# jimonld2000/AudioDenoiser

Hardware: AMD Instinct MI355X
Metric: spectrogram frames/sec (forward), 513x256 fp32 (higher is better)
Workload: dtype f32; 1 GPU; BASELINE configs[1]: batch=64 synthetic 513x256 fp32 spectrograms on one MI355X, full U-Net forward + per-clip perceptual loss; batch_per_gpu=64, global_batch=64, freq_bins=513, frames=256, parallelism=clips sharded over 1 rank(s), weights replicated, no data-path collective, lib_digest=ac1cc53c7748

## Files before the change

audiodenoiser_amd/csrc/adn_internal.h:

```cpp
#pragma once
#include <hip/hip_runtime.h>
#include <atomic>
#include <cstddef>
#include <cstdint>
#include <type_traits>

namespace adn {

template <typename T> constexpr int ACT_BLOCK = 32 / (int)sizeof(T);
template <typename T>
__host__ __device__ __forceinline__ long act_off(int C, long HW, long pix, int c)
{
    constexpr int B = ACT_BLOCK<T>;
    (void)C;
    return ((long)(c / B) * HW + pix) * B + (c % B);
}

#ifdef __HIPCC__
typedef float f32x2 __attribute__((ext_vector_type(2)));
typedef float f32x4 __attribute__((ext_vector_type(4)));
typedef float f32x16 __attribute__((ext_vector_type(16)));
typedef _Float16 f16x2 __attribute__((ext_vector_type(2)));
typedef _Float16 f16x4 __attribute__((ext_vector_type(4)));
typedef _Float16 f16x8 __attribute__((ext_vector_type(8)));
// ... 158 lines not shown
{
    const double out_mb = (double)out_floats * 4.0 * 1e-6;
    int best = 1;
    double tbest = 0.0;
    for (int ks = 1; ks <= ADN_MAX_KSPLIT; ks *= 2) {
        if (nchunk % ks || (ks > 1 && nchunk / ks < 8)) break;
        const double t = 8.0 + 1.28 * (nchunk / ks) * (double)((nwg * ks + 767) / 768) + (ks > 1 ? 4.0 + (ks + 1) * out_mb / 8.0 : 0.0);
        if (ks == 1 || t < tbest - 0.5) {
            best = ks;
            tbest = t;
        }
    }
    return best;
}

inline int conv16_ksplit(long nwg, int nchunk, size_t out_floats)
{
    if (nwg > 64) return 1;
    int ks = 1;
    while (ks < 8 && nwg * ks * 2 <= 256 && nchunk % (ks * 2) == 0 && nchunk / (ks * 2) >= 4 &&
           (size_t)(ks * 2) * out_floats * 4 <= ((size_t)32 << 20))
        ks *= 2;
    return ks;
}

enum ConvKind { CONV3X3_RELU = 0, CONV3X3_RELU_POOL = 1, CONVT2X2 = 2, CONV3X3_RELU_DOT = 3, WINO_GEMM = 4 };

struct ConvGeom {
    int TH;
    int BN;
    int KC;
};
ConvGeom conv_geom(ConvKind kind, int Cout, bool f16);
long conv_mfma_tiles(ConvKind kind, bool f16, ConvArgs &a);

template <auto... KERNELS>
hipError_t lds_opt_in(size_t bytes)
{
    static std::atomic<unsigned long long> done{0};
    int dev = 0;
    if (hipGetDevice(&dev) != hipSuccess) return hipErrorInvalidDevice;
    const unsigned long long bit = 1ull << (dev & 63);
    if (done.load(std::memory_order_acquire) & bit) return hipSuccess;
    for (const void *k : {reinterpret_cast<const void *>(KERNELS)...}) {
        const hipError_t e = hipFuncSetAttribute(k, hipFuncAttributeMaxDynamicSharedMemorySize, (int)bytes);
        if (e != hipSuccess) return e;
    }
    done.fetch_or(bit, std::memory_order_release);
    return hipSuccess;
}
inline int device_cus()
{
    static std::atomic<int> cus{0};
    int c = cus.load(std::memory_order_relaxed);
    if (c == 0) {
        int dev = 0;
        if (hipGetDevice(&dev) != hipSuccess || hipDeviceGetAttribute(&c, hipDeviceAttributeMultiprocessorCount, dev) != hipSuccess || c < 8)
            return 0;
        c &= ~7;
        cus.store(c, std::memory_order_relaxed);
    }
    return c;
}

hipError_t launch_conv_mfma(ConvKind kind, const ConvArgs &a, bool f16, hipStream_t st);
hipError_t launch_conv_reduce(ConvKind kind, const ConvArgs &a, bool f16, hipStream_t st);
hipError_t launch_convt_reduce(const float *partial, const float *bias, float *out, int ksplit, int N, int Ho, int Wo, int Cout,
                               hipStream_t st);
constexpr int WINO_BN = 32;
hipError_t launch_wino_conv(ConvKind kind, const ConvArgs &a, hipStream_t st);
long wino_tiles(ConvArgs &a);
bool wino4_applicable(ConvKind kind, const ConvArgs &a, bool force);
long wino4_workgroups(const ConvArgs &a);
hipError_t launch_wino4_conv(ConvKind kind, const ConvArgs &a, hipStream_t st);

struct Wino3sGeom {
    int tilesY, tilesX;
    long rows;
    size_t v_bytes, m_bytes;
    long gemm_grid;
};
bool wino3s_applicable(ConvKind kind, const ConvArgs &a);
Wino3sGeom wino3s_geom(const ConvArgs &a);
hipError_t launch_wino3s_conv(ConvKind kind, const ConvArgs &a, float *V, float *M, hipStream_t st);
hipError_t launch_wino_gemm(const float *V, const void *U, float *M, long rows, int Cin, int Cout, hipStream_t st);

bool conv16_applicable(ConvKind kind, const ConvArgs &a);
hipError_t launch_conv16(ConvKind kind, const ConvArgs &a, bool resident, hipStream_t st);

bool convt16_applicable(const ConvArgs &a);
hipError_t launch_convt16(const ConvArgs &a, hipStream_t st);

hipError_t launch_conv_first(const float *x, const float *w9x64, const float *bias, void *out, bool f16,
                             int N, int H, int W, int Cin, hipStream_t st);
hipError_t launch_dot_finish(const float *planes, int nplanes, float bias, float *y, long npix, hipStream_t st);
hipError_t launch_conv_out(const void *in, bool f16, const float *w64, float bias, float *out, long npix, long HW,
                           long out_stride, hipStream_t st);
hipError_t launch_nhwc_to_nchw(const void *in, bool f16, float *out, int N, int H, int W, int C, hipStream_t st);

hipError_t launch_stft_mag(const float *audio, int n_clips, long L, int n_fft, int hop, int center, long n_frames,
                           float *out, int rows, long row_stride, long clip_stride, int quantize, hipStream_t st);
constexpr hipError_t ADN_COLD_IN_CAPTURE = hipErrorStreamCaptureUnsupported;
bool stream_is_capturing(hipStream_t st);
hipError_t stft_tables(int n_fft, const float **out, hipStream_t st);
hipError_t loss_tables(hipStream_t st);
hipError_t launch_gl_polar(const float *mag, const float *rnd, int n_clips, int F, int T, void *spec, hipStream_t st);
hipError_t launch_istft_frames(const void *spec, int n_clips, int T, int n_fft, float *buf, hipStream_t st);
hipError_t launch_istft_ola(const float *buf, int n_clips, int T, int n_fft, int hop, float *audio, hipStream_t st);
hipError_t launch_stft_complex(const float *audio, int n_clips, long L, int n_fft, int hop, int T, void *spec,
                               hipStream_t st);
struct DenoiseGeom {
    int T, K, Wd, S, V;
};
bool denoise_geom(int n_frames, int window, int overlap, DenoiseGeom *g);
hipError_t launch_denoise_windows(const void *spec, int n_clips, int F, const DenoiseGeom &g, float *out, hipStream_t st);
hipError_t launch_denoise_stitch(const float *y, int n_clips, int F, const DenoiseGeom &g, int clamp, float *out,
                                 hipStream_t st);
hipError_t launch_denoise_resynth(const float *y, const void *spec, int n_clips, long L, int n_fft, int hop,
                                  const DenoiseGeom &g, float *audio, hipStream_t st);
struct SpectralConsts {
    float smooth, one_minus_smooth, beta, gamma, growth, alpha, one_minus_alpha, gain_floor, bias;
};
hipError_t launch_spectral_gain(const void *spec, int n_clips, int T, int F, const SpectralConsts &k, const float *state_in,
                                float *state_out, float *out, int width, int col0, hipStream_t st);
constexpr int SPECTRAL_MAX_ROWS = 256;
struct SpectralRow {
    int slot, fresh;
};
struct SpectralRows {
    int n;
    SpectralRow row[SPECTRAL_MAX_ROWS];
};
hipError_t launch_spectral_gain_windows(const float *windows, float *y, int n_rows, int n_steps, int F, int W, int col0, int n_cols,
                                        const SpectralConsts &k, float *state, const SpectralRows &rows, hipStream_t st);
struct WpeConsts {
    int K, D, I;
    float loading, rho;
};
long wpe_grid(int n_clips, int F, int K);
hipError_t launch_wpe(const void *spec, int n_clips, int T, int F, const WpeConsts &k, void *spec_out, float *mag_out, int width,
                      hipStream_t st);
struct StreamGeom {
    int n_fft, hop, W, B, A;
    int S, RX, RM;
    long x_off, mag_off, hist_off, tail_off, total;
};
struct StreamCall {
    int first, n_steps, T, L;
    int base, end, f_new0, f_new1;
    int slot_in, slot_out;
    int f_first, f_last, p_begin, p_first, p_out, p_tail, p_end;
};
__host__ __device__ inline StreamCall stream_call_of(const StreamGeom &g, long first, int n_steps, long final_length)
{
    StreamCall c;
    const long B = g.B, D = g.B + g.A, hop = g.hop, M = g.n_fft / 2, keep = g.n_fft - g.hop;
    const long last = first + n_steps - 1;
    c.first = (int)first;
    c.n_steps = n_steps;
    c.T = -1;
    c.L = -1;
    bool closes = false;
    if (final_length > 0) {
        const long T = 1 + final_length / hop, K = (T + B - 1) / B;
        c.T = (int)T;
        c.L = (int)final_length;
        closes = last == K - 1;
    }
// ... 117 lines not shown
```

audiodenoiser_amd/csrc/conv_kernels.hip:

```cpp
#include "adn_internal.h"

#include <cstdlib>

namespace adn {

namespace {

constexpr int TW = 16;
constexpr int CONVT_KG = 2, CONVT_WPE = 4;

template <typename T> struct Elem;
template <> struct Elem<float> { static constexpr int EPV = 4; };
template <> struct Elem<_Float16> { static constexpr int EPV = 8; };

template <int TH, int BN, int WM, int WN>
__device__ __forceinline__ void conv_epilogue_raw(const ConvArgs &p, f32x16 (&acc)[TH * TW / 32 / WM][BN / 32 / WN], int lane, int wave,
                                                  int ct, int n, int ty, int tx)
{
    constexpr int MB = TH * TW / 32 / WM, NB = BN / 32 / WN;
    const int wm = wave / WN, wn = wave % WN;
    const int hh = lane >> 5, l31 = lane & 31;
    float *ob = static_cast<float *>(p.out) + (size_t)n * p.H * p.W * p.Cout;
#pragma unroll
    for (int j = 0; j < NB; ++j) {
// ... 804 lines not shown
        for (int s = 1; s < ADN_MAX_KSPLIT; ++s)
            if (s < ksplit) v += t[s];
        v += bv;
        v.x = relu_nan(v.x); v.y = relu_nan(v.y); v.z = relu_nan(v.z); v.w = relu_nan(v.w);
        *reinterpret_cast<Tx4 *>(out + (size_t)n * img + act_off<T>(Cout, (long)H * W, (long)gy * W + gx, c4)) = as_t(v);
        return v;
    };
    if constexpr (!POOL) {
        finish(by, bx);
    } else {
        f32x4 mx = {0.f, 0.f, 0.f, 0.f};
#pragma unroll
        for (int a = 0; a < 2; ++a)
#pragma unroll
            for (int b = 0; b < 2; ++b) {
                const int gy = 2 * by + a, gx = 2 * bx + b;
                if (gy >= H || gx >= W) continue;
                const f32x4 v = finish(gy, gx);
                mx.x = max_nan(mx.x, v.x); mx.y = max_nan(mx.y, v.y); mx.z = max_nan(mx.z, v.z); mx.w = max_nan(mx.w, v.w);
            }
        if (by < H / 2 && bx < W / 2)
            *reinterpret_cast<Tx4 *>(pool + (size_t)n * (H / 2) * (W / 2) * Cout +
                                     act_off<T>(Cout, (long)(H / 2) * (W / 2), (long)by * (W / 2) + bx, c4)) = as_t(mx);
    }
}

template <typename T>
hipError_t launch_conv_mfma_t(ConvKind kind, const ConvArgs &a, hipStream_t st)
{
    if constexpr (sizeof(T) == 2) {
        if (a.ksplit > 1) {
            if (kind != CONV3X3_RELU) return hipErrorInvalidValue;
            return launch_dma_cfg<T, 32, 64, 8, 1, 9, 1, CONV3X3_RELU, 4, 0, 1>(a, st);
        }
        if (kind == CONVT2X2) return launch_dma_cfg<T, 8, 128, 2, 2, 1, CONVT_KG, CONVT2X2, CONVT_WPE>(a, st);
        if (kind == CONV3X3_RELU_DOT) {
            if (a.nct != 1 || !a.dotw || !a.dot_out) return hipErrorInvalidValue;
            return launch_dma_cfg<T, 32, 64, 8, 1, 9, 1, CONV3X3_RELU_DOT, 4>(a, st);
        }
        if (kind == CONV3X3_RELU_POOL) return launch_dma_cfg<T, 32, 64, 8, 1, 9, 1, CONV3X3_RELU_POOL, 4>(a, st);
        return launch_dma_cfg<T, 32, 64, 8, 1, 9, 1, CONV3X3_RELU, 4>(a, st);
    } else {
        if (kind == CONV3X3_RELU_DOT) return hipErrorInvalidValue;
        if (kind == CONVT2X2) {
            if (a.split && a.ksplit > 1) return launch_dma_cfg<T, 8, 128, 2, 2, 1, CONVT_KG, CONVT2X2, 3, 1, 1>(a, st);
            if (a.ksplit > 1) return hipErrorInvalidValue;
            if (a.split) return launch_dma_cfg<T, 8, 128, 2, 2, 1, CONVT_KG, CONVT2X2, 3, 1>(a, st);
            return launch_dma_cfg<T, 8, 128, 2, 2, 1, CONVT_KG, CONVT2X2, CONVT_WPE>(a, st);
        }
        if (a.Cout == 64) {
            if (kind == CONV3X3_RELU_POOL) return launch_cfg<T, 16, 64, 4, 1, 9, 1, CONV3X3_RELU_POOL>(a, st);
            return launch_cfg<T, 16, 64, 4, 1, 9, 1, CONV3X3_RELU>(a, st);
        }
        if (kind == CONV3X3_RELU_POOL) return launch_cfg<T, 8, 128, 2, 2, 9, 1, CONV3X3_RELU_POOL>(a, st);
        return launch_cfg<T, 8, 128, 2, 2, 9, 1, CONV3X3_RELU>(a, st);
    }
}

}

ConvGeom conv_geom(ConvKind kind, int Cout, bool f16)
{
    const int cpg = f16 ? 16 : 8;
    if (kind == CONVT2X2) return ConvGeom{8, 128, CONVT_KG * cpg};
    if (f16) return ConvGeom{32, 64, cpg};
    if (Cout == 64) return ConvGeom{16, 64, cpg};
    return ConvGeom{8, 128, cpg};
}

long conv_mfma_tiles(ConvKind kind, bool f16, ConvArgs &a)
{
    const ConvGeom g = conv_geom(kind, a.Cout, f16);
    a.tilesY = (a.H + g.TH - 1) / g.TH;
    a.tilesX = (a.W + TW - 1) / TW;
    a.nct = (kind == CONVT2X2 ? 4 * a.Cout : a.Cout) / g.BN;
    return conv_workgroups(a);
}

hipError_t launch_conv_mfma(ConvKind kind, const ConvArgs &a, bool f16, hipStream_t st)
{
    return f16 ? launch_conv_mfma_t<_Float16>(kind, a, st) : launch_conv_mfma_t<float>(kind, a, st);
}

hipError_t launch_wino_gemm(const float *V, const void *U, float *M, long rows, int Cin, int Cout, hipStream_t st)
{
    if (!V || !U || !M || rows < 1 || rows >= (1L << 25) || Cin < 16 || (Cin & 15) || Cout < 128 || (Cout & 127)) return hipErrorInvalidValue;
    ConvArgs a{};
    a.N = 36;
    a.W = TW;
    a.H = (int)((rows + TW - 1) / TW);
    a.rows = rows;
    a.s0 = ConvSrc{V, a.H, a.W, Cin, 0, 0};
    a.s1 = ConvSrc{V, 0, 0, 0, 0, 0};
    a.nchunk0 = a.nchunk = Cin / 16;
    a.wpk = U;
    a.out = M;
    a.Cout = Cout;
    a.ksplit = 1;
    a.split = 1;
    a.tilesY = (a.H + 7) / 8;
    a.tilesX = 1;
    a.nct = Cout / 128;
    return launch_dma_cfg<float, 8, 128, 2, 2, 1, CONVT_KG, WINO_GEMM, 3, 1>(a, st);
}

template <typename T>
static hipError_t launch_conv_reduce_t(bool pl, const ConvArgs &a, unsigned blocks, hipStream_t st)
{
    if (pl)
        hipLaunchKernelGGL((conv_reduce_kernel<T, true>), dim3(blocks), dim3(256), 0, st, a.partial, a.bias, static_cast<T *>(a.out),
                           static_cast<T *>(a.pool), a.ksplit, a.N, a.H, a.W, a.Cout);
    else
        hipLaunchKernelGGL((conv_reduce_kernel<T, false>), dim3(blocks), dim3(256), 0, st, a.partial, a.bias, static_cast<T *>(a.out),
                           static_cast<T *>(nullptr), a.ksplit, a.N, a.H, a.W, a.Cout);
    return hipGetLastError();
}

hipError_t launch_conv_reduce(ConvKind kind, const ConvArgs &a, bool f16, hipStream_t st)
{
    const bool pl = kind == CONV3X3_RELU_POOL;
    if (a.ksplit < 2 || a.ksplit > ADN_MAX_KSPLIT || !a.partial || (a.Cout & (f16 ? 15 : 3)) || (kind != CONV3X3_RELU && !pl) || (pl && !a.pool))
        return hipErrorInvalidValue;
    const long items = pl ? (long)a.N * ((a.H + 1) / 2) * ((a.W + 1) / 2) * (a.Cout / 4) : (long)a.N * a.H * a.W * (a.Cout / 4);
    const long blocks = (items + 255) / 256;
    if (items <= 0 || blocks > 0x7fffffffL) return hipErrorInvalidValue;
    return f16 ? launch_conv_reduce_t<_Float16>(pl, a, (unsigned)blocks, st) : launch_conv_reduce_t<float>(pl, a, (unsigned)blocks, st);
}

hipError_t launch_convt_reduce(const float *partial, const float *bias, float *out, int ksplit, int N, int Ho, int Wo, int Cout,
                               hipStream_t st)
{
    const long n4 = (long)N * Ho * Wo * Cout / 4;
    const long blocks = (n4 + 255) / 256;
    if (ksplit < 2 || ksplit > ADN_MAX_KSPLIT || (Cout & 7) || blocks <= 0 || blocks > 0x7fffffffL) return hipErrorInvalidValue;
    hipLaunchKernelGGL(convt_reduce_kernel, dim3((unsigned)blocks), dim3(256), 0, st, reinterpret_cast<const f32x4 *>(partial), bias,
                       reinterpret_cast<f32x4 *>(out), ksplit, n4, (long)Ho * Wo, Cout / 8);
    return hipGetLastError();
}

hipError_t launch_conv_first(const float *x, const float *w9x64, const float *bias, void *out, bool f16,
                             int N, int H, int W, int Cin, hipStream_t st)
{
    if (Cin < 1 || Cin > 64) return hipErrorInvalidValue;
    const int tiles_y = (H + FIRST_ROWS - 1) / FIRST_ROWS;
    const int max_cols = 4096 / Cin - 2;
    int tiles_x = (W + max_cols - 1) / max_cols;
    while ((long)N * tiles_y * tiles_x < 512 && (W + 2 * tiles_x - 1) / (2 * tiles_x) >= 64) tiles_x *= 2;
    const int cols = (W + tiles_x - 1) / tiles_x;
    tiles_x = (W + cols - 1) / cols;
    const long blocks = (long)N * tiles_y * tiles_x;
    const size_t lds = (size_t)Cin * (FIRST_ROWS + 2) * (cols + 2) * sizeof(float);
    if (blocks <= 0 || blocks > 0x7fffffffL || lds > 160 * 1024) return hipErrorInvalidValue;
    if (lds > 64 * 1024) {
        const void *fn = f16 ? reinterpret_cast<const void *>(conv_first_kernel<_Float16>)
                             : reinterpret_cast<const void *>(conv_first_kernel<float>);
        hipError_t e = hipFuncSetAttribute(fn, hipFuncAttributeMaxDynamicSharedMemorySize, (int)lds);
        if (e != hipSuccess) return e;
    }
    if (f16)
        hipLaunchKernelGGL(conv_first_kernel<_Float16>, dim3((unsigned)blocks), dim3(256), lds, st, x, w9x64, bias,
                           static_cast<_Float16 *>(out), H, W, tiles_y, tiles_x, cols, Cin);
    else
        hipLaunchKernelGGL(conv_first_kernel<float>, dim3((unsigned)blocks), dim3(256), lds, st, x, w9x64, bias,
                           static_cast<float *>(out), H, W, tiles_y, tiles_x, cols, Cin);
    return hipGetLastError();
}

hipError_t launch_conv_out(const void *in, bool f16, const float *w64, float bias, float *out, long npix, long HW,
// ... 36 lines not shown
```

audiodenoiser_amd/csrc/unet.hip:

```cpp
#include "adn_host.h"

#include <algorithm>
#include <cmath>
#include <cstdlib>
#include <cstring>
#include <memory>
#include <vector>

using adn::aligned_to;
using adn::DeviceGuard;
using adn::fail;
using adn::fail_hip;

namespace {

constexpr float BN_EPS = 1e-5f;
constexpr int CH[5] = {64, 128, 256, 512, 1024};

enum LayerKind { CONV3, CONVT };
struct LayerDesc {
    LayerKind kind;
    int level;
    int C0, C1;
    int Cout;
};
constexpr int N_CONV3 = 17, N_CONVT = 4, N_LAYERS = N_CONV3 + N_CONVT;
struct LayerTable {
    LayerDesc v[N_LAYERS];
    int n;
};
constexpr LayerTable make_layers()
{
    LayerTable t{};
    for (int l = 0; l <= 4; ++l) {
        if (l > 0) t.v[t.n++] = LayerDesc{CONV3, l, CH[l - 1], 0, CH[l]};
        t.v[t.n++] = LayerDesc{CONV3, l, CH[l], 0, CH[l]};
    }
    for (int l = 3; l >= 0; --l) {
        t.v[t.n++] = LayerDesc{CONVT, l + 1, CH[l + 1], 0, CH[l]};
        t.v[t.n++] = LayerDesc{CONV3, l, CH[l], CH[l], CH[l]};
        t.v[t.n++] = LayerDesc{CONV3, l, CH[l], 0, CH[l]};
    }
    return t;
}
constexpr LayerTable NET = make_layers();
static_assert(NET.n == N_LAYERS && NET.v[0].Cout == 64 && NET.v[8].C0 == 1024 && NET.v[9].kind == CONVT && NET.v[N_LAYERS - 1].Cout == 64,
              "layer table: 9 layers down to the bottleneck, then 4 x (convT, conv, conv)");
static_assert(6 * (1 + N_CONV3) + 2 * N_CONVT + 2 == ADN_N_WEIGHT_TENSORS, "layer table does not match the weight tensor list");
static_assert(1 + N_LAYERS + 1 == ADN_N_LAUNCHES, "layer table does not match the timing slots");

struct LayerWeights {
    size_t w_off, b_off;
    size_t w4_off;
    size_t w3_off;
    size_t w16_off;
    size_t braw_off;
};

}

struct adn_unet {
    int device = 0;
    float *dev = nullptr;
    size_t dev_floats = 0;
    size_t first_w = 0, first_b = 0;
    LayerWeights lw[N_LAYERS] = {};
    size_t out_w = 0;
    size_t zero_off = 0;
    float out_b = 0.f;
    std::vector<float> out_bias;
    int in_ch = 1, n_classes = 1;
    std::vector<hipEvent_t> events;
    int timing_max = 0, timing_count = 0;
    bool f16 = false;
    bool use_wino = true;
    bool use_wino4 = true, force_wino4 = false;
    bool allow_split = false;
    bool convt_split = true;
    int f16_conv = 1;
    int f16_convt = 1;
    bool f16_fuse_first = true;
    bool batch_invariant = false;
    long auto_grid = 192, auto_grid64 = 512;
    int wino_gemm = 1;
    long gemm_grid = 1536;
};

namespace {

void bn_fold(const float *b, const float *gamma, const float *beta, const float *mean, const float *var, int C,
             std::vector<float> &scale, std::vector<float> &bias)
{
    scale.resize(C);
    bias.resize(C);
    for (int c = 0; c < C; ++c) {
        const float s = gamma[c] / std::sqrt(var[c] + BN_EPS);
        scale[c] = s;
        bias[c] = (b[c] - mean[c]) * s + beta[c];
    }
}

template <typename T>
void pack_conv3x3(const float *w , const std::vector<float> &scale, int Cin, int Cout, T *dst)
{
    constexpr int EPV = 16 / sizeof(T);
    const adn::ConvGeom g = adn::conv_geom(adn::CONV3X3_RELU, Cout, sizeof(T) == 2);
    const int BN = g.BN, KC = g.KC, KG = KC / (2 * EPV);
    const int nct = Cout / BN, nchunk = Cin / KC;
    size_t o = 0;
    for (int ct = 0; ct < nct; ++ct)
        for (int ch = 0; ch < nchunk; ++ch)
            for (int tap = 0; tap < 9; ++tap)
                for (int s = 0; s < KG; ++s)
                    for (int h = 0; h < 2; ++h)
                        for (int n = 0; n < BN; ++n) {
                            const int co = ct * BN + n;
                            for (int kk = 0; kk < EPV; ++kk) {
                                const int ci = ch * KC + 2 * EPV * s + EPV * h + kk;
                                dst[o++] = (T)(w[((size_t)co * Cin + ci) * 9 + tap] * scale[co]);
                            }
                        }
}

void pack_conv16(const float *w , const std::vector<float> &scale, int Cin, int Cout, _Float16 *dst)
{
    const int nchunk = Cin / 32;
    for (int co = 0; co < Cout; ++co)
        for (int ci = 0; ci < Cin; ++ci) {
            const int ct = co / 64, j = (co % 64) / 16, c16 = co % 16, ch = ci / 32, g = (ci % 32) / 8, e = ci % 8;
            for (int tap = 0; tap < 9; ++tap)
                dst[(((((size_t)ct * nchunk + ch) * 9 + tap) * 4 + j) * 64 + g * 16 + c16) * 8 + e] =
                    (_Float16)(w[((size_t)co * Cin + ci) * 9 + tap] * scale[co]);
        }
}

void pack_wino3x3(const float *w , const std::vector<float> &scale, int Cin, int Cout, int BN,
                  float *dst)
{
    static const double G[4][3] = {{1, 0, 0}, {0.5, 0.5, 0.5}, {0.5, -0.5, 0.5}, {0, 0, 1}};
    const int nct = Cout / BN, nchunk = Cin / 8;
    for (int co = 0; co < Cout; ++co)
        for (int ci = 0; ci < Cin; ++ci) {
            const float *g = w + ((size_t)co * Cin + ci) * 9;
            double tmp[4][3], U[4][4];
            for (int x = 0; x < 4; ++x)
                for (int b = 0; b < 3; ++b)
                    tmp[x][b] = G[x][0] * g[0 * 3 + b] + G[x][1] * g[1 * 3 + b] + G[x][2] * g[2 * 3 + b];
            for (int x = 0; x < 4; ++x)
                for (int v = 0; v < 4; ++v)
                    U[x][v] = (tmp[x][0] * G[v][0] + tmp[x][1] * G[v][1] + tmp[x][2] * G[v][2]) * (double)scale[co];
            const int ct = co / BN, n = co % BN, ch = ci / 8, q = (ci % 8) / 2, e = ci & 1;
            float *blk = dst + ((size_t)ct * nchunk + ch) * (16 * 4 * BN * 2);
            for (int pos = 0; pos < 16; ++pos)
                blk[(((((pos >> 1) * (BN / 16) + n / 16) * 4 + q) * 16) + (n % 16)) * 4 + (pos & 1) * 2 + e] =
                    (float)U[pos >> 2][pos & 3];
        }
    (void)nct;
}

void wino4_u(const float *g , float scale, float (&U)[36])
{
    static const double G[6][3] = {{1.0 / 4, 0, 0},           {-1.0 / 6, -1.0 / 6, -1.0 / 6}, {-1.0 / 6, 1.0 / 6, -1.0 / 6},
                                   {1.0 / 24, 1.0 / 12, 1.0 / 6}, {1.0 / 24, -1.0 / 12, 1.0 / 6}, {0, 0, 1}};
    double tmp[6][3];
    for (int x = 0; x < 6; ++x)
        for (int b = 0; b < 3; ++b)
            tmp[x][b] = G[x][0] * g[0 * 3 + b] + G[x][1] * g[1 * 3 + b] + G[x][2] * g[2 * 3 + b];
    for (int x = 0; x < 6; ++x)
// ... 243 lines not shown
    const void *U = nullptr;
    float *V = nullptr, *M = nullptr;
    size_t v_bytes = 0, m_bytes = 0;
};
struct Conv3Choice {
    Conv3Kernel kernel;
    int ksplit;
    bool fuse_first;
    bool fuse_out;
};

Conv3Choice choose_conv3(const adn_unet *h, adn::ConvKind kind, const adn::ConvArgs &a, bool first = false, bool tail = false,
                         const WinoScratch &sc = WinoScratch())
{
    Conv3Choice c{DIRECT, 1, false, false};
    if (h->f16) {
        const bool c16 = a.wpk4 && adn::conv16_applicable(kind, a);
        c.fuse_out = tail && a.nct == 1;
        if (first && h->f16_fuse_first && c16) {
            c.kernel = CONV16;
            c.fuse_first = true;
            return c;
        }
        if (a.wpk4 && !h->batch_invariant && !c.fuse_out)
            c.ksplit = adn::conv16_ksplit(adn::conv_workgroups(a), a.nchunk, (size_t)a.N * a.H * a.W * a.Cout);
        if (c.ksplit == 1 && c16) c.kernel = CONV16;
        return c;
    }
    if (!h->use_wino) return c;
    c.kernel = WINO2;
    c.fuse_out = tail && a.nct == 2;
    auto done = [&]() {
        c.fuse_first = first && c.kernel == WINO2 && c.ksplit == 1;
        return c;
    };
    const bool can_split = !c.fuse_out;
    const bool f4_ok = a.wpk4 && adn::wino4_applicable(kind, a, h->force_wino4);
    const long g2 = adn::conv_workgroups(a);
    if (h->allow_split && can_split) {
        c.ksplit = adn::wino_ksplit(g2, a.nchunk);
        if (c.ksplit == 1 && f4_ok) c.kernel = WINO4;
        return done();
    }
    const bool automatic = !h->batch_invariant && !h->force_wino4;
    const long thr = a.Cout <= 64 ? h->auto_grid64 : h->auto_grid;
    const long g4 = f4_ok ? adn::wino4_workgroups(a) : 0;
    if (h->wino_gemm && sc.U && !c.fuse_out && !first && adn::wino3s_applicable(kind, a)) {
        const adn::Wino3sGeom g3 = adn::wino3s_geom(a);
        const bool fits = g3.v_bytes <= sc.v_bytes && g3.m_bytes <= sc.m_bytes;
        const bool pinned = h->batch_invariant && !h->force_wino4;
        if (fits && (h->wino_gemm == 2 || pinned || (automatic && g3.gemm_grid >= h->gemm_grid))) {
            c.kernel = WINO3S;
            return c;
        }
    }
    if (f4_ok && (!automatic || g4 >= thr)) {
        c.kernel = WINO4;
        return done();
    }
    if (automatic && can_split) c.ksplit = adn::wino_ksplit(g2, a.nchunk);
    if (automatic && can_split && f4_ok) {
        const int ks4 = adn::wino4_ksplit(g4, a.nchunk);
        if (ks4 > 1) {
            const double out_mb = (double)a.N * a.H * a.W * a.Cout * 4.0 * 1e-6;
            auto reduce_us = [&](int ks) { return ks > 1 ? 4.0 + (ks + 1) * out_mb / 8.0 : 0.0; };
            const double t4 = 12.0 + 2.79 * (a.nchunk / ks4) * (double)((g4 * ks4 + 255) / 256) + reduce_us(ks4);
            const double t2 = 8.0 + 2.06 * (a.nchunk / c.ksplit) * (double)((g2 * c.ksplit + 511) / 512) + reduce_us(c.ksplit);
            if (t4 < t2) {
                c.kernel = WINO4;
                c.ksplit = ks4;
            }
        }
    }
    return done();
}

hipError_t launch_conv3_kernels(const adn_unet *h, adn::ConvKind kind, const Conv3Choice &c, adn::ConvArgs a, float *partial, hipStream_t st,
                                const WinoScratch &sc)
{
    if (c.fuse_out) kind = adn::CONV3X3_RELU_DOT;
    switch (c.kernel) {
    case WINO3S:
        a.wpk = sc.U;
        return adn::launch_wino3s_conv(kind, a, sc.V, sc.M, st);
    case CONV16:
        a.wpk = a.wpk4;
        a.nchunk0 = a.s0.C / 32;
        a.nchunk = (a.s0.C + a.s1.C) / 32;
        if (c.fuse_first) a.nchunk0 = a.nchunk = 2;
        return adn::launch_conv16(kind, a, c.fuse_first || (a.s0.C + a.s1.C == 64 && a.Cout == 64), st);
    case DIRECT:
        if (c.ksplit > 1) {
            adn::ConvArgs sl = a;
            sl.ksplit = c.ksplit;
            sl.out = partial;
            sl.pool = nullptr;
            hipError_t e = adn::launch_conv_mfma(adn::CONV3X3_RELU, sl, true, st);
            if (e != hipSuccess) return e;
            a.ksplit = c.ksplit;
            a.partial = partial;
            return adn::launch_conv_reduce(kind, a, true, st);
        }
        return adn::launch_conv_mfma(kind, a, h->f16, st);
    case WINO4:
        a.wpk = a.wpk4;
        [[fallthrough]];
    case WINO2:
        a.ksplit = c.ksplit;
        a.partial = partial;
        return c.kernel == WINO4 ? adn::launch_wino4_conv(kind, a, st) : adn::launch_wino_conv(kind, a, st);
    }
    return hipErrorInvalidValue;
}

inline int hip_status(hipError_t e, const char *what)
{
    return e == hipSuccess ? ADN_OK : fail_hip(e, what);
}

int check_part(int layer, int ks, size_t out_floats, size_t part_bytes)
{
    if (ks <= 1 || (size_t)ks * out_floats * sizeof(float) <= part_bytes) return ADN_OK;
    const LayerDesc &d = NET.v[layer];
    return fail(ADN_ERR_WORKSPACE, "adn_unet_forward: layer " + std::to_string(layer) + " (" + (d.kind == CONVT ? "transposed convolution" : "3x3 convolution") +
                " at level " + std::to_string(d.level) + ", " + std::to_string(d.C0 + d.C1) + " -> " + std::to_string(d.Cout) + " channels): " +
                std::to_string(ks) + " K-split copies of " + std::to_string(out_floats * sizeof(float)) + " bytes do not fit the " +
                std::to_string(part_bytes) + " bytes the workspace plan reserves for them");
}

int launch_conv3(const adn_unet *h, int layer, adn::ConvKind kind, const Conv3Choice &c, adn::ConvArgs a, float *partial, size_t part_bytes,
                 hipStream_t st, const WinoScratch &sc = WinoScratch())
{
    if (int rc = check_part(layer, c.ksplit, (size_t)a.N * a.H * a.W * a.Cout, part_bytes)) return rc;
    return hip_status(launch_conv3_kernels(h, kind, c, a, partial, st, sc), "launch_conv3");
}

struct ConvTChoice {
    bool t16;
    int ksplit;
};

ConvTChoice choose_convt(const adn_unet *h, const LayerWeights &L, const adn::ConvArgs &a)
{
    ConvTChoice c{false, 1};
    if (h->f16) {
        c.t16 = L.w16_off && adn::convt16_applicable(a);
        return c;
    }
    if (h->convt_split && !h->batch_invariant)
        c.ksplit = adn::convt_ksplit(adn::conv_workgroups(a), a.nchunk, (size_t)a.N * (2 * a.H) * (2 * a.W) * a.Cout);
    return c;
}

hipError_t launch_convt_kernels(const adn_unet *h, const LayerWeights &L, const ConvTChoice &c, adn::ConvArgs a, float *partial, hipStream_t st)
{
    if (c.t16) {
        a.wpk = h->dev + L.w16_off;
        a.bias = h->dev + L.braw_off;
        return adn::launch_convt16(a, st);
    }
    if (c.ksplit > 1) {
        float *out = static_cast<float *>(a.out);
        a.ksplit = c.ksplit;
        a.out = partial;
        a.bias = h->dev + h->zero_off;
        hipError_t e = adn::launch_conv_mfma(adn::CONVT2X2, a, h->f16, st);
        if (e != hipSuccess) return e;
// ... 98 lines not shown
    void *X = tB, *Y = tA;
    Conv3Choice last{};
    for (int l = 3; l >= 0; --l) {
        const adn::ConvArgs t = convt_args(h, p, i++, X, Y);
        ADN_MARK();
        ADN_TRY(launch_convt(h, i - 1, choose_convt(h, h->lw[i - 1], t), t, part, p.part_bytes, st));
        const WinoScratch sa = wino_scratch(i);
        const adn::ConvArgs a = conv_args(h, p, i++, ws + p.skip[l], Y, 2 * t.H, 2 * t.W, X, nullptr);
        ADN_MARK();
        ADN_TRY(launch_conv3(h, i - 1, adn::CONV3X3_RELU, choose_conv3(h, adn::CONV3X3_RELU, a, false, false, sa), a, part, p.part_bytes, st, sa));
        const WinoScratch sb = wino_scratch(i);
        adn::ConvArgs b = conv_args(h, p, i++, X, nullptr, 0, 0, Y, nullptr);
        last = choose_conv3(h, adn::CONV3X3_RELU, b, false, l == 0 && !taps && h->n_classes == 1, sb);
        if (last.fuse_out) {
            b.dotw = h->dev + h->out_w;
            b.dot_out = f16 ? y : static_cast<float *>(Y);
            if (f16) b.dot_bias = h->out_b;
        }
        ADN_MARK();
        ADN_TRY(launch_conv3(h, i - 1, adn::CONV3X3_RELU, last, b, part, p.part_bytes, st, sb));
        ADN_HIP(export_tap(5 + (3 - l), Y, i - 1));
        std::swap(X, Y);
    }
    ADN_MARK();
    if (last.fuse_out && f16) {
    } else if (last.fuse_out)
        ADN_HIP(adn::launch_dot_finish(static_cast<const float *>(X), 2, h->out_b, y, (long)N * F * T, st));
    else
        for (int k = 0; k < h->n_classes; ++k)
            ADN_HIP(adn::launch_conv_out(X, f16, h->dev + h->out_w + (size_t)64 * k, h->out_bias[k], y + (size_t)k * F * T,
                                         (long)N * F * T, (long)F * T, (long)h->n_classes * F * T, st));
    ADN_MARK();
    if (timed) {
        if (evi != ADN_N_LAUNCHES + 1) return fail(ADN_ERR_INVALID, "internal: launch count mismatch");
        ++h->timing_count;
    }
#undef ADN_MARK
#undef ADN_TRY
    if (taps && taps[9])
        ADN_HIP(hipMemcpyAsync(taps[9], y, (size_t)N * h->n_classes * F * T * sizeof(float), hipMemcpyDeviceToDevice, st));
    return ADN_OK;
}


int check_create_args(adn_unet **handle, int device, const float *const *t, int n_tensors, int dtype, int in_channels, int num_classes)
{
    if (!handle || !t) return fail(ADN_ERR_INVALID, "adn_unet_create: null argument");
    if (in_channels < 1 || in_channels > 64 || num_classes < 1 || num_classes > 64)
        return fail(ADN_ERR_INVALID, "adn_unet_create_general: need 1 <= in_channels <= 64 and 1 <= num_classes <= 64");
    if (dtype != ADN_DTYPE_F32 && dtype != ADN_DTYPE_F16) return fail(ADN_ERR_INVALID, "adn_unet_create: dtype must be ADN_DTYPE_F32 or ADN_DTYPE_F16");
    if (n_tensors != ADN_N_WEIGHT_TENSORS) return fail(ADN_ERR_INVALID, "adn_unet_create: expected 118 tensors");
    for (int i = 0; i < n_tensors; ++i)
        if (!t[i]) return fail(ADN_ERR_INVALID, "adn_unet_create: null tensor pointer");
    int ndev = 0;
    if (hipGetDeviceCount(&ndev) != hipSuccess || ndev <= 0) return fail(ADN_ERR_NO_DEVICE, "no HIP device visible");
    if (device < 0 || device >= ndev) return fail(ADN_ERR_INVALID, "adn_unet_create: bad device index");
    return ADN_OK;
}

int check_device_arch(int device)
{
    hipDeviceProp_t prop;
    ADN_HIP(hipGetDeviceProperties(&prop, device));
    if (std::strncmp(prop.gcnArchName, "gfx950", 6) != 0)
        return fail(ADN_ERR_NO_DEVICE, std::string("libadn is built for gfx950 only, device is ") + prop.gcnArchName);
    return ADN_OK;
}

void read_switches(adn_unet &h)
{
    if (const char *algo = std::getenv("ADN_CONV_ALGO"))
        h.use_wino = std::strcmp(algo, "direct") != 0;
    if (h.f16) h.use_wino = false;
    if (const char *sk = std::getenv("ADN_WINO_SPLITK")) h.allow_split = std::atoi(sk) != 0;
    if (const char *cs = std::getenv("ADN_CONVT_SPLIT")) h.convt_split = std::atoi(cs) != 0;
    if (const char *bi = std::getenv("ADN_BATCH_INVARIANT")) h.batch_invariant = std::atoi(bi) != 0;
    if (const char *ff = std::getenv("ADN_F16_FIRST")) h.f16_fuse_first = std::atoi(ff) != 0;
    if (const char *fc = std::getenv("ADN_F16_CONV")) h.f16_conv = std::atoi(fc) == 32 ? 0 : 1;
    if (const char *ft = std::getenv("ADN_F16_CONVT")) h.f16_convt = std::strcmp(ft, "dma") == 0 ? 0 : 1;
    if (const char *ag = std::getenv("ADN_AUTO_GRID")) h.auto_grid = std::atol(ag);
    if (const char *ag = std::getenv("ADN_AUTO_GRID64")) h.auto_grid64 = std::atol(ag);
    if (h.f16) h.convt_split = false;
    if (const char *wg = std::getenv("ADN_WINO_GEMM")) h.wino_gemm = std::atoi(wg) == 2 ? 2 : std::atoi(wg) != 0;
    if (const char *wt = std::getenv("ADN_WINO_TILE")) {
        h.use_wino4 = std::atoi(wt) != 2;
        h.force_wino4 = std::atoi(wt) == 4;
    }
}

void pack_weights(adn_unet &h, const float *const *t, std::vector<float> &host)
{
    auto reserve = [&](size_t n) {
        const size_t at = host.size();
        host.resize(at + ((n + 63) & ~size_t(63)), 0.f);
        return at;
    };
    auto halfs = [&](size_t off) { return reinterpret_cast<_Float16 *>(host.data() + off); };
    std::vector<float> scale, bias;
    bn_fold(t[1], t[2], t[3], t[4], t[5], 64, scale, bias);
    h.first_w = reserve((size_t)h.in_ch * 9 * 64);
    for (int ci = 0; ci < h.in_ch; ++ci)
        for (int tap = 0; tap < 9; ++tap)
            for (int co = 0; co < 64; ++co)
                host[h.first_w + ((size_t)ci * 9 + tap) * 64 + co] = t[0][((size_t)co * h.in_ch + ci) * 9 + tap] * scale[co];
    h.first_b = reserve(64);
    std::memcpy(host.data() + h.first_b, bias.data(), sizeof(float) * 64);
    int ti = 6;
    for (int i = 0; i < N_LAYERS; ++i) {
        const LayerDesc &d = NET.v[i];
        LayerWeights &L = h.lw[i];
        const int Cin = d.C0 + d.C1, Cout = d.Cout;
        const size_t n16 = ((size_t)(d.kind == CONVT ? 4 : 9) * Cin * Cout + 1) / 2;
        if (d.kind == CONVT) {
            if (h.f16) {
                L.w_off = reserve(n16);
                pack_convt<_Float16>(t[ti], Cin, Cout, halfs(L.w_off));
                if (h.f16_convt != 0 && Cin % 128 == 0 && Cout % 64 == 0) {
                    L.w16_off = reserve(n16);
                    pack_convt16(t[ti], Cin, Cout, halfs(L.w16_off));
                    L.braw_off = reserve(Cout);
                    std::memcpy(host.data() + L.braw_off, t[ti + 1], sizeof(float) * Cout);
                }
            } else if (h.convt_split) {
                L.w_off = reserve(3 * n16);
                pack_convt_split(t[ti], Cin, Cout, reinterpret_cast<uint16_t *>(host.data() + L.w_off));
                L.braw_off = reserve(Cout);
                std::memcpy(host.data() + L.braw_off, t[ti + 1], sizeof(float) * Cout);
            } else {
                L.w_off = reserve((size_t)4 * Cin * Cout);
                pack_convt<float>(t[ti], Cin, Cout, host.data() + L.w_off);
            }
            L.b_off = reserve((size_t)4 * Cout);
            for (int col = 0; col < 4 * Cout; ++col) {
                int ij, c;
                adn::convt_column(col, Cout, ij, c);
                host[L.b_off + col] = t[ti + 1][c];
            }
            ti += 2;
            continue;
        }
        bn_fold(t[ti + 1], t[ti + 2], t[ti + 3], t[ti + 4], t[ti + 5], Cout, scale, bias);
        if (h.f16 && h.f16_conv != 0 && Cin % 32 == 0 && Cout % 64 == 0) {
            L.w16_off = reserve(n16);
            pack_conv16(t[ti], scale, Cin, Cout, halfs(L.w16_off));
        }
        if (h.use_wino) {
            L.w_off = reserve((size_t)16 * Cin * Cout);
            pack_wino3x3(t[ti], scale, Cin, Cout, adn::WINO_BN, host.data() + L.w_off);
            if (h.use_wino4) {
                L.w4_off = reserve((size_t)36 * Cin * Cout);
                pack_wino4_3x3(t[ti], scale, Cin, Cout, host.data() + L.w4_off);
                if (h.wino_gemm && d.level >= 3 && Cin >= 512 && Cin % 16 == 0 && Cout % 128 == 0) {
                    L.w3_off = reserve((size_t)36 * Cin * Cout * 3 / 2);
                    pack_wino4_split(t[ti], scale, Cin, Cout, reinterpret_cast<uint16_t *>(host.data() + L.w3_off));
                }
            }
        } else if (h.f16) {
            L.w_off = reserve(n16);
            pack_conv3x3<_Float16>(t[ti], scale, Cin, Cout, halfs(L.w_off));
        } else {
            L.w_off = reserve((size_t)9 * Cin * Cout);
            pack_conv3x3<float>(t[ti], scale, Cin, Cout, host.data() + L.w_off);
        }
        L.b_off = reserve(Cout);
        std::memcpy(host.data() + L.b_off, bias.data(), sizeof(float) * Cout);
        ti += 6;
// ... 129 lines not shown
```

audiodenoiser_amd/csrc/wino3s_kernels.hip:

```cpp
#include "adn_internal.h"

namespace adn {

namespace {

constexpr int NT = 256;

__global__ __launch_bounds__(NT) void wino3s_input_kernel(const ConvArgs p, float *__restrict__ V, int tilesY, int tilesX, long rows)
{
    const long id = (long)blockIdx.x * NT + threadIdx.x;
    const long row = id >> 1;
    const int half = (int)(id & 1), cb = blockIdx.y;
    if (row >= rows) return;
    const int tx = (int)(row % tilesX);
    const long r2 = row / tilesX;
    const int ty = (int)(r2 % tilesY), n = (int)(r2 / tilesY);
    const bool second = cb >= p.s0.C / 8;
    const ConvSrc &s = second ? p.s1 : p.s0;
    const int cbl = second ? cb - p.s0.C / 8 : cb;
    const float *src = static_cast<const float *>(s.ptr) + ((size_t)n * (s.C / 8) + cbl) * ((size_t)s.H * s.W * 8) + half * 4;
    const int y0 = 4 * ty - 1 - s.offY, x0 = 4 * tx - 1 - s.offX;
    f32x4 d[6][6];
#pragma unroll
    for (int a = 0; a < 6; ++a)
// ... 12 lines not shown
    const size_t pstr = (size_t)ncb * rows * 8;
#pragma unroll
    for (int i = 0; i < 6; ++i)
#pragma unroll
        for (int j = 0; j < 6; ++j) *reinterpret_cast<f32x4 *>(vp + (size_t)(6 * i + j) * pstr) = d[i][j];
}

template <bool POOL>
__global__ __launch_bounds__(NT) void wino3s_output_kernel(const ConvArgs p, const float *__restrict__ M, int tilesY, int tilesX,
                                                           long rows)
{
    const long id = (long)blockIdx.x * NT + threadIdx.x;
    const long row = id >> 1;
    const int half = (int)(id & 1), cb = blockIdx.y;
    if (row >= rows) return;
    const int tx = (int)(row % tilesX);
    const long r2 = row / tilesX;
    const int ty = (int)(r2 % tilesY), n = (int)(r2 / tilesY);
    const float *mp = M + ((size_t)cb * rows + row) * 8 + half * 4;
    const size_t pstr = (size_t)(p.Cout / 8) * rows * 8;
    f32x4 w[4][6];
#pragma unroll
    for (int j = 0; j < 6; ++j) {
        f32x4 m[6];
#pragma unroll
        for (int i = 0; i < 6; ++i) m[i] = *reinterpret_cast<const f32x4 *>(mp + (size_t)(6 * i + j) * pstr);
        at6(m[0], m[1], m[2], m[3], m[4], m[5], w[0][j], w[1][j], w[2][j], w[3][j]);
    }
    const f32x4 bias = *reinterpret_cast<const f32x4 *>(p.bias + cb * 8 + half * 4);
    const f32x4 zero = {0.f, 0.f, 0.f, 0.f};
    f32x4 y[4][4];
#pragma unroll
    for (int a = 0; a < 4; ++a) {
        at6(w[a][0], w[a][1], w[a][2], w[a][3], w[a][4], w[a][5], y[a][0], y[a][1], y[a][2], y[a][3]);
#pragma unroll
        for (int b = 0; b < 4; ++b) y[a][b] = __builtin_elementwise_maximum(y[a][b] + bias, zero);
    }
    float *ob = static_cast<float *>(p.out) + ((size_t)n * (p.Cout / 8) + cb) * ((size_t)p.H * p.W * 8) + half * 4;
#pragma unroll
    for (int a = 0; a < 4; ++a)
#pragma unroll
        for (int b = 0; b < 4; ++b) {
            const int gy = 4 * ty + a, gx = 4 * tx + b;
            if (gy < p.H && gx < p.W) *reinterpret_cast<f32x4 *>(ob + ((size_t)gy * p.W + gx) * 8) = y[a][b];
        }
    if constexpr (POOL) {
        const int Hp = p.H >> 1, Wp = p.W >> 1;
        float *pb = static_cast<float *>(p.pool) + ((size_t)n * (p.Cout / 8) + cb) * ((size_t)Hp * Wp * 8) + half * 4;
#pragma unroll
        for (int a = 0; a < 2; ++a)
#pragma unroll
            for (int b = 0; b < 2; ++b) {
                const int py = 2 * ty + a, px = 2 * tx + b;
                const f32x4 mx = __builtin_elementwise_maximum(__builtin_elementwise_maximum(y[2 * a][2 * b], y[2 * a][2 * b + 1]),
                                                               __builtin_elementwise_maximum(y[2 * a + 1][2 * b], y[2 * a + 1][2 * b + 1]));
                if (py < Hp && px < Wp) *reinterpret_cast<f32x4 *>(pb + ((size_t)py * Wp + px) * 8) = mx;
            }
    }
}

}

bool wino3s_applicable(ConvKind kind, const ConvArgs &a)
{
    if (kind != CONV3X3_RELU && kind != CONV3X3_RELU_POOL) return false;
    if (kind == CONV3X3_RELU_POOL && !a.pool) return false;
    const int Cin = a.s0.C + a.s1.C;
    if (a.firstw || a.ksplit > 1 || Cin < 16 || (Cin & 15) || (a.s0.C & 7) || a.Cout < 128 || (a.Cout & 127)) return false;
    return a.N >= 1 && a.H >= 1 && a.W >= 1 && wino3s_geom(a).rows < (1L << 25);
}

Wino3sGeom wino3s_geom(const ConvArgs &a)
{
    Wino3sGeom g{};
    g.tilesY = (a.H + 3) / 4;
    g.tilesX = (a.W + 3) / 4;
    g.rows = (long)a.N * g.tilesY * g.tilesX;
    g.v_bytes = (size_t)36 * g.rows * (a.s0.C + a.s1.C) * sizeof(float);
    g.m_bytes = (size_t)36 * g.rows * a.Cout * sizeof(float);
    g.gemm_grid = 36 * ((g.rows + 127) / 128) * (a.Cout / 128);
    return g;
}

hipError_t launch_wino3s_conv(ConvKind kind, const ConvArgs &a, float *V, float *M, hipStream_t st)
{
    if (!wino3s_applicable(kind, a) || !V || !M || !a.wpk || !a.bias || !a.out) return hipErrorInvalidValue;
    const Wino3sGeom g = wino3s_geom(a);
    const long bx = (2 * g.rows + NT - 1) / NT;
    const int Cin = a.s0.C + a.s1.C;
    hipLaunchKernelGGL(wino3s_input_kernel, dim3((unsigned)bx, (unsigned)(Cin / 8)), dim3(NT), 0, st, a, V, g.tilesY, g.tilesX, g.rows);
    hipError_t e = hipGetLastError();
    if (e != hipSuccess) return e;
    e = launch_wino_gemm(V, a.wpk, M, g.rows, Cin, a.Cout, st);
    if (e != hipSuccess) return e;
    if (kind == CONV3X3_RELU_POOL)
        hipLaunchKernelGGL(wino3s_output_kernel<true>, dim3((unsigned)bx, (unsigned)(a.Cout / 8)), dim3(NT), 0, st, a, M, g.tilesY,
                           g.tilesX, g.rows);
    else
        hipLaunchKernelGGL(wino3s_output_kernel<false>, dim3((unsigned)bx, (unsigned)(a.Cout / 8)), dim3(NT), 0, st, a, M, g.tilesY,
                           g.tilesX, g.rows);
    return hipGetLastError();
}

}
```

Measured before the change: 510,900 frames/s.

## Add 256x256-tile bf16x3 MFMA kernel for Winograd batched GEMM

Adds a dedicated Winograd-domain GEMM kernel that uses 256x256 output tiles with 512 threads, a triple-buffered LDS ring fed by buffer-load-to-LDS DMA, and a bf16x3 split-precision MFMA scheme. It is selected automatically when Cout is a multiple of 256 and the grid still fills all CUs, with an env override to force either tile size. The larger tile is meant to raise arithmetic intensity and operand reuse per fetched byte compared with the 128-wide generic path. The cost is higher LDS and register use per workgroup, hence lower occupancy, and fewer workgroups for small layers.

Result: no change. 512,400 frames/s, median of 6 (+0.3%).

```diff
diff --git a/audiodenoiser_amd/csrc/adn_internal.h b/audiodenoiser_amd/csrc/adn_internal.h
--- a/audiodenoiser_amd/csrc/adn_internal.h
+++ b/audiodenoiser_amd/csrc/adn_internal.h
@@ -264,8 +264,11 @@
 };
 bool wino3s_applicable(ConvKind kind, const ConvArgs &a);
 Wino3sGeom wino3s_geom(const ConvArgs &a);
-hipError_t launch_wino3s_conv(ConvKind kind, const ConvArgs &a, float *V, float *M, hipStream_t st);
-hipError_t launch_wino_gemm(const float *V, const void *U, float *M, long rows, int Cin, int Cout, hipStream_t st);
+hipError_t launch_wino3s_conv(ConvKind kind, const ConvArgs &a, float *V, float *M, hipStream_t st, int gemm_tile = 0);
+hipError_t launch_wino_gemm(const float *V, const void *U, float *M, long rows, int Cin, int Cout, hipStream_t st, int tile = 0);
+bool wino_gemm256_applicable(long rows, int Cin, int Cout);
+long wino_gemm256_grid(long rows, int Cout);
+hipError_t launch_wino_gemm256(const float *V, const void *U, float *M, long rows, int Cin, int Cout, hipStream_t st);
 
 bool conv16_applicable(ConvKind kind, const ConvArgs &a);
 hipError_t launch_conv16(ConvKind kind, const ConvArgs &a, bool resident, hipStream_t st);
diff --git a/audiodenoiser_amd/csrc/conv_kernels.hip b/audiodenoiser_amd/csrc/conv_kernels.hip
--- a/audiodenoiser_amd/csrc/conv_kernels.hip
+++ b/audiodenoiser_amd/csrc/conv_kernels.hip
@@ -910,8 +910,13 @@
     return f16 ? launch_conv_mfma_t<_Float16>(kind, a, st) : launch_conv_mfma_t<float>(kind, a, st);
 }
 
-hipError_t launch_wino_gemm(const float *V, const void *U, float *M, long rows, int Cin, int Cout, hipStream_t st)
-{
+hipError_t launch_wino_gemm(const float *V, const void *U, float *M, long rows, int Cin, int Cout, hipStream_t st, int tile)
+{
+    if (tile != 128 && wino_gemm256_applicable(rows, Cin, Cout)) {
+        const int cus = device_cus();
+        if (cus == 0) return hipErrorInvalidDevice;
+        if (tile == 256 || wino_gemm256_grid(rows, Cout) >= cus) return launch_wino_gemm256(V, U, M, rows, Cin, Cout, st);
+    }
     if (!V || !U || !M || rows < 1 || rows >= (1L << 25) || Cin < 16 || (Cin & 15) || Cout < 128 || (Cout & 127)) return hipErrorInvalidValue;
     ConvArgs a{};
     a.N = 36;
diff --git a/audiodenoiser_amd/csrc/unet.hip b/audiodenoiser_amd/csrc/unet.hip
--- a/audiodenoiser_amd/csrc/unet.hip
+++ b/audiodenoiser_amd/csrc/unet.hip
@@ -84,6 +84,7 @@
     long auto_grid = 192, auto_grid64 = 512;
     int wino_gemm = 1;
     long gemm_grid = 1536;
+    int wino_gemm_tile = 0;
 };
 
 namespace {
@@ -493,7 +494,7 @@
     switch (c.kernel) {
     case WINO3S:
         a.wpk = sc.U;
-        return adn::launch_wino3s_conv(kind, a, sc.V, sc.M, st);
+        return adn::launch_wino3s_conv(kind, a, sc.V, sc.M, st, h->wino_gemm_tile);
     case CONV16:
         a.wpk = a.wpk4;
         a.nchunk0 = a.s0.C / 32;
@@ -758,6 +759,7 @@
     if (const char *ag = std::getenv("ADN_AUTO_GRID64")) h.auto_grid64 = std::atol(ag);
     if (h.f16) h.convt_split = false;
     if (const char *wg = std::getenv("ADN_WINO_GEMM")) h.wino_gemm = std::atoi(wg) == 2 ? 2 : std::atoi(wg) != 0;
+    if (const char *gt = std::getenv("ADN_WINO_GEMM_TILE")) h.wino_gemm_tile = std::atoi(gt) == 128 ? 128 : std::atoi(gt) == 256 ? 256 : 0;
     if (const char *wt = std::getenv("ADN_WINO_TILE")) {
         h.use_wino4 = std::atoi(wt) != 2;
         h.force_wino4 = std::atoi(wt) == 4;
diff --git a/audiodenoiser_amd/csrc/wino3s_kernels.hip b/audiodenoiser_amd/csrc/wino3s_kernels.hip
--- a/audiodenoiser_amd/csrc/wino3s_kernels.hip
+++ b/audiodenoiser_amd/csrc/wino3s_kernels.hip
@@ -118,7 +118,7 @@
     return g;
 }
 
-hipError_t launch_wino3s_conv(ConvKind kind, const ConvArgs &a, float *V, float *M, hipStream_t st)
+hipError_t launch_wino3s_conv(ConvKind kind, const ConvArgs &a, float *V, float *M, hipStream_t st, int gemm_tile)
 {
     if (!wino3s_applicable(kind, a) || !V || !M || !a.wpk || !a.bias || !a.out) return hipErrorInvalidValue;
     const Wino3sGeom g = wino3s_geom(a);
@@ -127,7 +127,7 @@
     hipLaunchKernelGGL(wino3s_input_kernel, dim3((unsigned)bx, (unsigned)(Cin / 8)), dim3(NT), 0, st, a, V, g.tilesY, g.tilesX, g.rows);
     hipError_t e = hipGetLastError();
     if (e != hipSuccess) return e;
-    e = launch_wino_gemm(V, a.wpk, M, g.rows, Cin, a.Cout, st);
+    e = launch_wino_gemm(V, a.wpk, M, g.rows, Cin, a.Cout, st, gemm_tile);
     if (e != hipSuccess) return e;
     if (kind == CONV3X3_RELU_POOL)
         hipLaunchKernelGGL(wino3s_output_kernel<true>, dim3((unsigned)bx, (unsigned)(a.Cout / 8)), dim3(NT), 0, st, a, M, g.tilesY,
diff --git a/audiodenoiser_amd/csrc/wino_gemm_kernels.hip b/audiodenoiser_amd/csrc/wino_gemm_kernels.hip
--- /dev/null
+++ b/audiodenoiser_amd/csrc/wino_gemm_kernels.hip
@@ -0,0 +1,178 @@
+#include "adn_internal.h"
+
+namespace adn {
+
+namespace {
+
+constexpr int G_NT = 512;
+constexpr int G_ROWS = 256, G_COLS = 256;
+constexpr int G_V_BYTES = 2 * G_ROWS * 32;
+constexpr int G_SLAB = 3 * 2 * 128 * 16;
+constexpr int G_U_BYTES = 2 * G_SLAB;
+constexpr int G_IMG = G_V_BYTES + G_U_BYTES;
+constexpr int G_NBUF = 3;
+constexpr size_t G_LDS = (size_t)G_NBUF * G_IMG;
+constexpr int G_RS = 72;
+static_assert(8 * 32 * G_RS * 4 <= (int)G_LDS, "staging tiles of the eight waves fit the ring");
+
+struct WinoGemmArgs {
+    const float *V;
+    const void *U;
+    float *M;
+    long rows;
+    int Cout, nchunk;
+    int nct, nrt;
+};
+
+__global__ __launch_bounds__(G_NT, 2) void wino_gemm_bf16x3(const WinoGemmArgs p)
+{
+    extern __shared__ __attribute__((aligned(16))) char smem[];
+    const int tid = threadIdx.x;
+    const int lane = tid & 63;
+    const int wave = __builtin_amdgcn_readfirstlane(tid >> 6);
+    const int hh = lane >> 5, l31 = lane & 31;
+
+    int lid = __builtin_amdgcn_readfirstlane(xcd_remap((int)blockIdx.x, (int)gridDim.x));
+    const int ct = lid % p.nct;
+    lid /= p.nct;
+    const int rt = lid % p.nrt, pos = lid / p.nrt;
+    const int nchunk = p.nchunk;
+    const long rows = p.rows;
+
+    const unsigned vblk = (unsigned)(rows * 32);
+    const char *vpos = reinterpret_cast<const char *>(p.V) + (size_t)pos * (size_t)(2 * nchunk) * vblk;
+    const long vrow = (long)rt * G_ROWS + (tid >> 1);
+    const unsigned voff = vrow < rows ? (unsigned)vrow * 32u + (unsigned)(tid & 1) * 16u : ADN_DMA_OOB;
+    const unsigned ustr = (unsigned)nchunk * (unsigned)G_SLAB;
+    const __amdgpu_buffer_rsrc_t urs =
+        dma_rsrc(static_cast<const char *>(p.U) + ((size_t)pos * (2 * p.nct) + 2 * ct) * ustr, 2u * ustr);
+    auto fetch = [&](int c, int buf) {
+        const unsigned kill = c < nchunk ? 0u : ADN_DMA_OOB;
+        const int cc = c < nchunk ? c : nchunk - 1;
+        char *img = smem + buf * G_IMG;
+#pragma unroll
+        for (int k = 0; k < 2; ++k) {
+            const unsigned long long ab = reinterpret_cast<unsigned long long>(vpos) + (unsigned long long)(2 * cc + k) * vblk;
+            const unsigned lo = (unsigned)__builtin_amdgcn_readfirstlane((int)(unsigned)ab);
+            const unsigned hi = (unsigned)__builtin_amdgcn_readfirstlane((int)(unsigned)(ab >> 32));
+            __builtin_amdgcn_raw_ptr_buffer_load_lds(dma_rsrc(reinterpret_cast<const void *>(((unsigned long long)hi << 32) | lo), vblk),
+                                                     (__attribute__((address_space(3))) void *)(img + k * (G_V_BYTES / 2) + wave * 1024), 16,
+                                                     voff | kill, 0u, 0, 0);
+        }
+#pragma unroll
+        for (int k = 0; k < 3; ++k) {
+            const int sb = k * G_NT + wave * 64;
+            const int s = sb >= G_SLAB / 16 ? 1 : 0;
+            const unsigned soff = (unsigned)s * ustr + (unsigned)cc * (unsigned)G_SLAB + (unsigned)(sb - s * (G_SLAB / 16)) * 16u;
+            dma16_buf(urs, (unsigned)(lane * 16) | kill, (unsigned)__builtin_amdgcn_readfirstlane((int)soff),
+                      reinterpret_cast<float *>(img + G_V_BYTES + sb * 16));
+        }
+    };
+    fetch(0, 0);
+    fetch(1, 1);
+
+    f32x16 acc[8];
+#pragma unroll
+    for (int j = 0; j < 8; ++j)
+#pragma unroll
+        for (int r = 0; r < 16; ++r) acc[j][r] = 0.f;
+
+    const int a_lane = hh * (G_V_BYTES / 2) + (32 * wave + l31) * 32;
+    const int b_lane = G_V_BYTES + hh * 2048 + l31 * 16;
+
+    auto load_b = [&](const char *img, int j, bf16x8 (&b)[3]) {
+        const char *bp = img + b_lane + (j >> 2) * G_SLAB + (j & 3) * 512;
+#pragma unroll
+        for (int t = 0; t < 3; ++t) b[t] = __builtin_bit_cast(bf16x8, *reinterpret_cast<const f32x4 *>(bp + t * 4096));
+    };
+    auto mma6 = [&](f32x16 &d, const bf16x8 &ah, const bf16x8 &am, const bf16x8 &al, const bf16x8 (&b)[3]) {
+        d = __builtin_amdgcn_mfma_f32_32x32x16_bf16(al, b[0], d, 0, 0, 0);
+        d = __builtin_amdgcn_mfma_f32_32x32x16_bf16(ah, b[2], d, 0, 0, 0);
+        d = __builtin_amdgcn_mfma_f32_32x32x16_bf16(am, b[1], d, 0, 0, 0);
+        d = __builtin_amdgcn_mfma_f32_32x32x16_bf16(am, b[0], d, 0, 0, 0);
+        d = __builtin_amdgcn_mfma_f32_32x32x16_bf16(ah, b[1], d, 0, 0, 0);
+        d = __builtin_amdgcn_mfma_f32_32x32x16_bf16(ah, b[0], d, 0, 0, 0);
+    };
+
+    asm volatile("s_waitcnt vmcnt(5)" ::: "memory");
+    asm volatile("s_barrier" ::: "memory");
+
+    bf16x8 ah, am, al;
+    split3_bf16(*reinterpret_cast<const f32x4 *>(smem + a_lane), *reinterpret_cast<const f32x4 *>(smem + a_lane + 16), ah, am, al);
+    int par = 0;
+#pragma clang loop unroll(disable)
+    for (int c = 0; c < nchunk; ++c) {
+        fetch(c + 2, par == 0 ? 2 : par - 1);
+        const char *img = smem + par * G_IMG;
+        bf16x8 b[2][3];
+        load_b(img, 0, b[0]);
+#pragma unroll
+        for (int j = 0; j < 6; ++j) {
+            load_b(img, j + 1, b[(j + 1) & 1]);
+            mma6(acc[j], ah, am, al, b[j & 1]);
+        }
+        load_b(img, 7, b[1]);
+        par = par == 2 ? 0 : par + 1;
+        asm volatile("s_waitcnt vmcnt(5) lgkmcnt(0)" ::: "memory");
+        asm volatile("s_barrier" ::: "memory");
+        const char *nimg = smem + par * G_IMG;
+        const f32x4 x0 = *reinterpret_cast<const f32x4 *>(nimg + a_lane), x1 = *reinterpret_cast<const f32x4 *>(nimg + a_lane + 16);
+        mma6(acc[6], ah, am, al, b[0]);
+        mma6(acc[7], ah, am, al, b[1]);
+        split3_bf16(x0, x1, ah, am, al);
+    }
+    asm volatile("s_waitcnt vmcnt(0) lgkmcnt(0)" ::: "memory");
+    asm volatile("s_barrier" ::: "memory");
+
+    float *stage = reinterpret_cast<float *>(smem) + wave * (32 * G_RS);
+    const int srow = lane >> 1, shalf = lane & 1;
+    const long grow = (long)rt * G_ROWS + 32 * wave + srow;
+    float *mp = p.M + ((size_t)pos * (p.Cout / 8) + (size_t)ct * (G_COLS / 8)) * (size_t)rows * 8 + (size_t)grow * 8 + shalf * 4;
+#pragma unroll
+    for (int q = 0; q < 4; ++q) {
+#pragma unroll
+        for (int jj = 0; jj < 2; ++jj)
+#pragma unroll
+            for (int r = 0; r < 16; ++r)
+                stage[((r & 3) + 8 * (r >> 2) + 4 * hh) * G_RS + jj * 32 + l31] = acc[2 * q + jj][r] + 0.f;
+        asm volatile("s_waitcnt lgkmcnt(0)" ::: "memory");
+        f32x4 v[8];
+#pragma unroll
+        for (int b = 0; b < 8; ++b) v[b] = *reinterpret_cast<const f32x4 *>(stage + srow * G_RS + b * 8 + shalf * 4);
+        asm volatile("s_waitcnt lgkmcnt(0)" ::: "memory");
+        if (grow < rows) {
+#pragma unroll
+            for (int b = 0; b < 8; ++b) *reinterpret_cast<f32x4 *>(mp + (size_t)(q * 8 + b) * (size_t)rows * 8) = v[b];
+        }
+    }
+}
+
+}
+
+bool wino_gemm256_applicable(long rows, int Cin, int Cout)
+{
+    if (rows < 1 || rows >= (1L << 25) || Cin < 16 || (Cin & 15) || Cout < 256 || (Cout & 255)) return false;
+    return (size_t)2 * (Cin / 16) * G_SLAB < (size_t)0xfffffff0u && wino_gemm256_grid(rows, Cout) <= 0x7fffffffL;
+}
+
+long wino_gemm256_grid(long rows, int Cout) { return 36 * ((rows + G_ROWS - 1) / G_ROWS) * (Cout / G_COLS); }
+
+hipError_t launch_wino_gemm256(const float *V, const void *U, float *M, long rows, int Cin, int Cout, hipStream_t st)
+{
+    if (!V || !U || !M || !wino_gemm256_applicable(rows, Cin, Cout)) return hipErrorInvalidValue;
+    WinoGemmArgs a{};
+    a.V = V;
+    a.U = U;
+    a.M = M;
+    a.rows = rows;
+    a.Cout = Cout;
+    a.nchunk = Cin / 16;
+    a.nct = Cout / G_COLS;
+    a.nrt = (int)((rows + G_ROWS - 1) / G_ROWS);
+    const hipError_t e = lds_opt_in<wino_gemm_bf16x3>(G_LDS);
+    if (e != hipSuccess) return e;
+    hipLaunchKernelGGL(wino_gemm_bf16x3, dim3((unsigned)wino_gemm256_grid(rows, Cout)), dim3(G_NT), G_LDS, st, a);
+    return hipGetLastError();
+}
+
+}
```
